# baumlin/rebvio

Hardware: AMD Instinct MI355X
Metric: frames/sec at 640x480 (~15k keylines); 1-GPU and 8-stream/8-GPU batch (higher is better)
Workload: dtype f32; 1 GPU; 640x480 synthetic stream, ~15k keylines, detect+track+IRLS pose, fp32; streams=1, keylines=14942, frames_in_hbm=24, settle_frames=995, pairs_tracked_in_window=1144, parallelism=1 independent streams, 1 per GPU, rank0_numa_node=0

## Files before the change

rebvio_amd/csrc/api.hip:

```cpp
#include <chrono>
#include <cmath>
#include <cstdio>
#include <cstdlib>
#include <cstring>
#include <limits>
#include <atomic>
#include <condition_variable>
#include <deque>
#include <map>
#include <memory>
#include <mutex>
#include <shared_mutex>
#include <thread>
#include <string>
#include <vector>

#include "common.hpp"
#include "glue.hpp"
#include "hostmath.hpp"
#include "pixel_format.hpp"

using namespace rh;

namespace {
// ... 196 lines not shown
  rebvio_hip_pair_out out;
  int keylines;
};

struct PairQueue {
  struct Step {
    rebvio_hip_map* nm[kMaxLanes];
    uint32_t seq = 0;
    int slot = -1;
    int ev_slot = -1;
  };
  Step ring[kPairSlots];
  int head = 0, count = 0;
  Step& operator[](int i) { return ring[(head + i) % kPairSlots]; }
  void push_back(const Step& st) { ring[(head + count++) % kPairSlots] = st; }
  void pop_front() {
    head = (head + 1) % kPairSlots;
    --count;
  }
  std::deque<PairRec> done;
  hipEvent_t slot_ev[kPairSlots]{};
  double t_wait = 0;
};

struct rebvio_hip_ctx {
  std::shared_ptr<LifeBlock> life = std::make_shared<LifeBlock>();
  rebvio_hip_params P{};
  KParams K{};
  int device = 0;
  hipStream_t s_det{}, s_key{}, s_trk{};
  double t_begin_enq = 0, t_begin_wait = 0;
  uint64_t t_begin_n = 0;
  std::mutex dl_mu;
  float* sa2[2][2] = {{nullptr, nullptr}, {nullptr, nullptr}};
  float* dog2[kDetPar]{};
  float* mag2[kDetPar]{};
  int* rowcount2[kDetPar]{};
  hipEvent_t ev_scan[2]{};
  hipEvent_t prev_ready[2]{};
  uint64_t launch_index = 0;
  uint64_t release_counter = 0;
  ScaleBufs sb{};
  DetectBufs db{};
  DetState* det = nullptr;
  uint64_t frame_index = 0;
  rebvio_hip_map* last_detected = nullptr;
  int widths[2][3]{};
  std::vector<rebvio_hip_map*> pool;
  float* img_dev = nullptr;
  uint8_t* img8_dev = nullptr;
  static constexpr int kPin = 16;
  void* pin[kPin]{};
  hipEvent_t pin_ev[kPin]{};
  bool pin_used[kPin]{};
  uint64_t pin_next = 0;
  int2* undist_map = nullptr;
  float* undist_img[kDetPar]{};
  uint8_t* dmask_buf = nullptr;
  const uint8_t* dmask = nullptr;
  rebvio_hip_batch* batch = nullptr;
  rebvio_hip_keyline* aos_dev = nullptr;
  int* scratch_i = nullptr;
  float* diag0 = nullptr;
  float* diag1 = nullptr;
  LmState* lm = nullptr;
  float* part = nullptr;
  float* xrv_part = nullptr;
  int* hist = nullptr;
  float* fscratch = nullptr;
  int maxblocks = 0;
  unsigned long long* lm_xch = nullptr;
  unsigned lm_tag_base = 0;
// ... 24 lines not shown
  int lm_threads = 512;
  int dm_head_form = 0;
  static constexpr int kSlots = kPairSlots;
  PairSlot* slot[kSlots]{};
  GlueRec* rec[kSlots]{};
  GlueDev* glue_dev = nullptr;
  GlueStage* glue_stage = nullptr;
  GlueState* gstate = nullptr;
  GlueState* h_gstate = nullptr;
  hm::M3 gs_R{};
  int min_pool = 0;
  int lead = 5;
  int group = 4;
  uint32_t stamp_seq = 0;
  uint32_t last_stamp = 0;
  bool forge_stamp = false;
  std::mutex pool_mu;
  std::vector<rebvio_hip_map*> frames;
  PairQueue q;
  uint64_t pair_seq = 0;
  struct DetJob {
    rebvio_hip_map* m;
    const void* img;
    int is_u8;
    const DetState* det_in;
    DetState* det_out;
    const MapState* prev_st;
    int pin_slot = -1;
    size_t pin_bytes = 0;
    int fmt = 0;
    const uint8_t* mask_static = nullptr;
    const uint8_t* mask_frame = nullptr;
  };
  std::mutex det_mu;
  std::string det_error;
  double t_detect_enq = 0, t_enq = 0, t_queued = 0;
  double t_det_launch = 0;
  uint64_t t_det_n = 0;
  bool dbg = false;
  hm::M3 wbg_shadow{};
  bool wbg_shadow_valid = false;
  bool gyro_pre_on = true;
  uint64_t t_frames = 0;
  bool owns_streams = true;
  rebvio_hip_map* bf_map[2] = {nullptr, nullptr};
  bool bf_have[2] = {false, false};
  bool bf_copy_queued[2] = {false, false};
  hipEvent_t bf_done[2]{};
  MapState* h_bf = nullptr;
  int bf_cur = 0;
  int bf_res = -1;
  bool bf_nan[2] = {false, false};
};

namespace {
void release_map(rebvio_hip_map* m, hipEvent_t done_ref = nullptr, bool record_done = true);

inline bool map_dead(const rebvio_hip_map* m) { return !m || !m->life || m->life->dead.load(std::memory_order_acquire); }
class MapAlive {
 public:
  explicit MapAlive(const rebvio_hip_map* m) : hold_(m ? m->life : nullptr) {
    if (hold_) lock_ = std::shared_lock<std::shared_mutex>(hold_->mu);
    dead_ = map_dead(m);
    if (dead_) g_err = "the map's context has been destroyed (rebvio_hip_destroy)";
  }
  bool dead() const { return dead_; }
// ... 162 lines not shown
  DetectBufs db = c->db;
  db.rowcount = c->rowcount2[b];
  if (j.pin_slot >= 0) {
    launch_copy_from_pinned(c->s_det, c->pin[j.pin_slot], const_cast<void*>(j.img), j.pin_bytes);
    HIPCHK(hipEventRecord(c->pin_ev[j.pin_slot], c->s_det));
  }
  if (c->prev_ready[b]) HIPCHK(hipStreamWaitEvent(c->s_det, c->prev_ready[b], 0));
  const void* img = j.img;
  int is_u8 = j.is_u8;
  int fmt = is_u8 ? j.fmt : 0;
  if (is_u8 && c->undist_map) {
    if (fmt == px::GRAY8)
      launch_front_end_u8(c->s_det, c->K, (const uint8_t*)img, c->undist_map, c->undist_img[b]);
    else
      launch_front_end_px(c->s_det, c->K, (const uint8_t*)img, fmt, c->undist_map, c->undist_img[b]);
    img = c->undist_img[b];
    is_u8 = 0;
    fmt = 0;
  }
  launch_scale_space(c->s_det, c->K, img, is_u8, sb, c->widths, db.rowcount, 1, fmt);
  HIPCHK(hipEventRecord(c->ev_scan[b], c->s_det));
  HIPCHK(hipStreamWaitEvent(c->s_key, c->ev_scan[b], 0));
  launch_scale_space(c->s_key, c->K, img, is_u8, sb, c->widths, db.rowcount, 2);
  if (m->has_done) HIPCHK(hipStreamWaitEvent(c->s_key, m->done_ref ? m->done_ref : m->done, 0));
  launch_keylines(c->s_key, c->K, sb, db, m->d, j.det_in, j.det_out, j.prev_st, c->widths, j.mask_static, j.mask_frame);
  HIPCHK(hipGetLastError());
  launch_df_build(c->s_key, c->K, m->d, j.det_out, true);
  HIPCHK(hipGetLastError());
  HIPCHK(hipEventRecord(m->ready, c->s_key));
  c->prev_ready[b] = m->ready;
  return 0;
}

int detect_prepare(rebvio_hip_ctx* c, const void* img_dev, int is_u8, uint64_t ts, rebvio_hip_ctx::DetJob* job, int fmt = 0,
                   const uint8_t* mask_frame = nullptr) {
  rebvio_hip_map* m = acquire_map(c);
  if (!m) return fail_msg("edge-map pool exhausted (release maps or raise map_pool)", -2);
  m->ts = ts;
  m->df_built = true;
  m->raster_order = true;
  job->m = m;
  job->img = img_dev;
  job->is_u8 = is_u8;
  job->fmt = fmt;
  job->mask_static = c->dmask;
  job->mask_frame = mask_frame;
  job->det_in = c->det + (c->frame_index % kDetRing);
  job->det_out = c->det + ((c->frame_index + 1) % kDetRing);
  job->prev_st = c->last_detected ? c->last_detected->d.st : nullptr;
  c->frame_index++;
  c->last_detected = m;
  return 0;
}

void detect_failed(rebvio_hip_ctx* c, const rebvio_hip_ctx::DetJob& job) {
  {
    std::lock_guard<std::mutex> lk(c->det_mu);
    if (c->det_error.empty()) c->det_error = g_err.empty() ? std::string("detect launch failed") : g_err;
  }
  release_map(job.m, nullptr);
}

int stage_host_frame(rebvio_hip_ctx* c, const void* img, size_t pitch_bytes, size_t row_bytes, int* slot_out, size_t* bytes_out);

int detect(rebvio_hip_ctx* c, const void* img_dev, int is_u8, int fmt, uint64_t ts, rebvio_hip_map** out, const void* host = nullptr,
           size_t pitch_bytes = 0, size_t row_bytes = 0, const uint8_t* mask_frame = nullptr) {
  {
    std::lock_guard<std::mutex> lk(c->det_mu);
    if (!c->det_error.empty()) return fail_msg(c->det_error.c_str(), -8);
  }
  rebvio_hip_ctx::DetJob job;
  int rc = host ? stage_host_frame(c, host, pitch_bytes, row_bytes, &job.pin_slot, &job.pin_bytes) : 0;
  if (rc) return rc;
  rc = detect_prepare(c, img_dev, is_u8, ts, &job, fmt, mask_frame);
  if (rc) return rc;
  const auto t0 = std::chrono::steady_clock::now();
  rc = detect_launch(c, job);
  if (c->dbg) {
    c->t_det_launch += std::chrono::duration<double, std::micro>(std::chrono::steady_clock::now() - t0).count();
    c->t_det_n++;
  }
  if (rc) {
    detect_failed(c, job);
    return rc;
  }
  *out = job.m;
  return 0;
}

void rotate_inputs(const rebvio_hip_ctx* c, const float vel[3], const float Rvel[9], const float Rback[9], float vel_r[3],
                   float Rvel_r[9]) {
  (void)c;
  const hm::M3 Rb = hm::load3(Rback);
  hm::mulv(Rb, vel, vel_r);
  hm::store3(hm::mul(hm::mul(Rb, hm::load3(Rvel)), hm::transpose(Rb)), Rvel_r);
}

void sum_xrv(const float* h_xrv, int nblocks, float Wx[36], float JtF[6], int* nm) {
  double acc[28];
  for (int k = 0; k < 28; ++k) acc[k] = 0.0;
  for (int b = 0; b < nblocks; ++b)
    for (int k = 0; k < 28; ++k) acc[k] += (double)h_xrv[(size_t)b * kXrvStride + k];
  int k = 0;
  for (int i = 0; i < 6; ++i)
    for (int j = i; j < 6; ++j) {
      Wx[i * 6 + j] = (float)acc[k];
      Wx[j * 6 + i] = (float)acc[k];
      ++k;
    }
  for (int i = 0; i < 6; ++i) JtF[i] = (float)acc[21 + i];
  if (nm) *nm = (int)std::lround(acc[27]);
}

// ... 400 lines not shown
    c->lm_persistent = std::strcmp(e, "percall") != 0;
    c->lm_spec = std::strcmp(e, "seq") != 0;
    c->lm_spec_forced = std::strcmp(e, "spec") == 0 || std::strcmp(e, "spec3") == 0;
    c->lm_spec_forced_kf = std::strcmp(e, "spec3") == 0 ? 3 : 2;
    if (std::strncmp(e, "mix", 3) == 0) c->lm_mix = std::max(1, std::atoi(e + 3));
  }
  HIPCHK(hipMalloc(&c->lm, 16 * sizeof(LmState)));
  HIPCHK(hipMemset(c->lm, 0, 16 * sizeof(LmState)));
  HIPCHK(hipMalloc(&c->part, (size_t)(kMaxLmCalls + 1) * part_call_stride(c) * sizeof(float)));
  HIPCHK(hipMemset(c->part, 0, (size_t)(kMaxLmCalls + 1) * part_call_stride(c) * sizeof(float)));
  HIPCHK(hipMalloc(&c->xrv_part, (size_t)c->maxblocks * kXrvStride * sizeof(float)));
  HIPCHK(hipMalloc(&c->hist, 128 * sizeof(int)));
  HIPCHK(hipMemset(c->hist, 0, 128 * sizeof(int)));
  HIPCHK(hipMalloc(&c->lm_zero, sizeof(LmState)));
  HIPCHK(hipMemset(c->lm_zero, 0, sizeof(LmState)));
  for (int i = 0; i < rebvio_hip_ctx::kSlots; ++i) {
    const size_t sz = sizeof(PairSlot) + (size_t)c->maxblocks * kXrvStride * sizeof(float);
    HIPCHK(hipHostMalloc(&c->slot[i], sz, hipHostMallocDefault));
    std::memset(c->slot[i], 0, sz);
    HIPCHK(hipHostMalloc(&c->rec[i], sizeof(GlueRec), hipHostMallocDefault));
    std::memset(c->rec[i], 0, sizeof(GlueRec));
    HIPCHK(hipEventCreateWithFlags(&c->q.slot_ev[i], hipEventDisableTiming));
  }
  HIPCHK(hipMalloc(&c->fscratch, 64 * sizeof(float)));
  HIPCHK(hipMalloc(&c->glue_dev, rebvio_hip_ctx::kSlots * sizeof(GlueDev)));
  HIPCHK(hipMemset(c->glue_dev, 0, rebvio_hip_ctx::kSlots * sizeof(GlueDev)));
  HIPCHK(hipMalloc(&c->glue_stage, rebvio_hip_ctx::kSlots * sizeof(GlueStage)));
  HIPCHK(hipMemset(c->glue_stage, 0, rebvio_hip_ctx::kSlots * sizeof(GlueStage)));
  HIPCHK(hipMalloc(&c->gstate, 2 * sizeof(GlueState)));
  HIPCHK(hipMemset(c->gstate, 0, 2 * sizeof(GlueState)));
  HIPCHK(hipHostMalloc(&c->h_gstate, 2 * sizeof(GlueState), hipHostMallocDefault));
  if (const char* l = std::getenv("REBVIO_HIP_LEAD")) c->lead = std::min(12, std::max(3, std::atoi(l)));
  if (const char* g = std::getenv("REBVIO_HIP_GROUP")) c->group = std::min(6, std::max(1, std::atoi(g)));
  if (const char* e = std::getenv("REBVIO_HIP_LM_THREADS")) {
    const int v = std::atoi(e);
    if (v == 256 || v == 512 || v == 1024) c->lm_threads = v;
  }
  if (const char* e = std::getenv("REBVIO_HIP_DM_HEAD"))
    c->dm_head_form = dm_form_by_name(e);
  HIPCHK(hipHostMalloc(&c->h_lm, 2 * sizeof(LmState), hipHostMallocDefault));
  HIPCHK(hipHostMalloc(&c->h_part, part_call_stride(c) * sizeof(float), hipHostMallocDefault));
  HIPCHK(hipHostMalloc(&c->h_xrv, (size_t)c->maxblocks * kXrvStride * sizeof(float), hipHostMallocDefault));
  HIPCHK(hipHostMalloc(&c->h_st, 2 * sizeof(MapState), hipHostMallocDefault));
  HIPCHK(hipHostMalloc(&c->h_f, 64 * sizeof(float), hipHostMallocDefault));

  int pool = p->map_pool > 0 ? p->map_pool : 6;
  if (pool < 4) pool = 4;
  for (int i = 0; i < pool; ++i) {
    rebvio_hip_map* m = new rebvio_hip_map;
    m->ctx = c;
    m->life = c->life;
    c->pool.push_back(m);
    int rc = alloc_map(c, m);
    if (rc) return rc;
  }
  rebvio_hip_reset_state(c);
  c->dbg = std::getenv("REBVIO_HIP_DEBUG") != nullptr;
  if (const char* e = std::getenv("REBVIO_HIP_GYRO_PRE")) c->gyro_pre_on = e[0] != '0';
  HIPCHK(hipDeviceSynchronize());
  guard.c = nullptr;
  *out = c;
  return 0;
}

void rebvio_hip_destroy(rebvio_hip_ctx* c) {
  if (!c) return;
  const std::shared_ptr<LifeBlock> life = c->life;
  std::unique_lock<std::shared_mutex> life_lk(life->mu);
  residency_remove(c->device, c);
  (void)hipSetDevice(c->device);
  if (std::getenv("REBVIO_HIP_DEBUG") && c->t_begin_n)
    std::fprintf(stderr, "[rebvio_hip] track_pair_begin over %llu pairs (us): enqueue %.1f  wait for the first half %.1f\n",
                 (unsigned long long)c->t_begin_n, c->t_begin_enq / c->t_begin_n, c->t_begin_wait / c->t_begin_n);
  (void)hipDeviceSynchronize();
  {
    std::lock_guard<std::mutex> g(g_prof.mu);
    g_prof.drain();
  }
  for (auto* m : c->frames) m->in_use = false;
  life->dead.store(true, std::memory_order_release);
  for (auto* m : c->pool) {
    free_map_device(m);
    if (!m->in_use) delete m;
  }
  c->pool.clear();
  void* dptr[] = {c->sb.a[0], c->sb.a[1], c->sb.b[0], c->sb.b[1], c->sb.dog, c->sb.mag, c->db.stash, c->db.bits,
                  c->db.rowcount, c->det, c->img_dev, c->img8_dev, c->aos_dev, c->scratch_i, c->diag0, c->diag1, c->lm,
                  c->part, c->xrv_part, c->hist, c->fscratch, c->dmask_buf};
  for (void* p : dptr)
    if (p) (void)hipFree(p);
  for (int f = 0; f < 2; ++f)
    if (c->sa2[1][f]) (void)hipFree(c->sa2[1][f]);
  void* hptr[] = {c->h_lm, c->h_part, c->h_xrv, c->h_st, c->h_f};
  for (void* p : hptr)
    if (p) (void)hipHostFree(p);
  if (c->owns_streams) {
    if (c->s_det) (void)hipStreamDestroy(c->s_det);
    if (c->s_trk) (void)hipStreamDestroy(c->s_trk);
    if (c->s_key) (void)hipStreamDestroy(c->s_key);
  }
  for (int i = 0; i < 2; ++i) {
    if (c->ev_scan[i]) (void)hipEventDestroy(c->ev_scan[i]);
  }
  for (int i = 1; i < kDetPar; ++i) {
    if (c->dog2[i]) (void)hipFree(c->dog2[i]);
    if (c->mag2[i]) (void)hipFree(c->mag2[i]);
    if (c->rowcount2[i]) (void)hipFree(c->rowcount2[i]);
  }
  for (int i = 0; i < rebvio_hip_ctx::kSlots; ++i) {
    if (c->slot[i]) (void)hipHostFree(c->slot[i]);
    if (c->rec[i]) (void)hipHostFree(c->rec[i]);
    if (c->q.slot_ev[i]) (void)hipEventDestroy(c->q.slot_ev[i]);
  }
  if (c->gstate) (void)hipFree(c->gstate);
  if (c->h_gstate) (void)hipHostFree(c->h_gstate);
  if (c->undist_map) (void)hipFree(c->undist_map);
  for (int i = 0; i < kDetPar; ++i)
    if (c->undist_img[i]) (void)hipFree(c->undist_img[i]);
  if (c->lm_xch) (void)hipFree(c->lm_xch);
  for (int i = 0; i < rebvio_hip_ctx::kPin; ++i) {
    if (c->pin[i]) (void)hipHostFree(c->pin[i]);
    if (c->pin_ev[i]) (void)hipEventDestroy(c->pin_ev[i]);
  }
  if (c->glue_dev) (void)hipFree(c->glue_dev);
  if (c->glue_stage) (void)hipFree(c->glue_stage);
// ... 93 lines not shown
}

int rebvio_hip_front_end_u8(rebvio_hip_ctx* c, const uint8_t* img, float* out) {
  HIPCHK(hipSetDevice(c->device));
  if (!c->undist_map) return fail_msg("front_end_u8: no distortion model set (rebvio_hip_set_undistort)", -3);
  const size_t Pn = (size_t)c->P.rows * c->P.cols;
  HIPCHK(hipMemcpyAsync(c->img8_dev, img, Pn, hipMemcpyHostToDevice, c->s_det));
  launch_front_end_u8(c->s_det, c->K, c->img8_dev, c->undist_map, c->undist_img[0]);
  HIPCHK(hipGetLastError());
  HIPCHK(hipMemcpyAsync(out, c->undist_img[0], Pn * sizeof(float), hipMemcpyDeviceToHost, c->s_det));
  HIPCHK(hipStreamSynchronize(c->s_det));
  return 0;
}

int rebvio_hip_front_end_px(rebvio_hip_ctx* c, const void* img, size_t pitch_bytes, int fmt, float* out) {
  int rc = check_px(c, "front_end_px", img, fmt, true, pitch_bytes);
  if (rc) return rc;
  if (!out) return fail_msg("front_end_px: null output", -3);
  HIPCHK(hipSetDevice(c->device));
  if (!c->undist_map) return fail_msg("front_end_px: no distortion model set (rebvio_hip_set_undistort)", -3);
  const size_t Pn = (size_t)c->P.rows * c->P.cols;
  const size_t rowb = (size_t)c->P.cols * px::bytes_per_pixel(fmt);
  uint8_t* stage = static_cast<uint8_t*>(u8_staging(c, fmt));
  HIPCHK(hipMemcpy2DAsync(stage, rowb, img, pitch_bytes ? pitch_bytes : rowb, rowb, (size_t)c->P.rows, hipMemcpyHostToDevice, c->s_det));
  launch_front_end_px(c->s_det, c->K, stage, fmt, c->undist_map, c->undist_img[0]);
  HIPCHK(hipGetLastError());
  HIPCHK(hipMemcpyAsync(out, c->undist_img[0], Pn * sizeof(float), hipMemcpyDeviceToHost, c->s_det));
  HIPCHK(hipStreamSynchronize(c->s_det));
  return 0;
}

int rebvio_hip_detector_state(rebvio_hip_ctx* c, float* threshold, float* auto_threshold, int* count) {
  HIPCHK(hipSetDevice(c->device));
  HIPCHK(hipStreamSynchronize(c->s_det));
  HIPCHK(hipStreamSynchronize(c->s_key));
  DetState d;
  HIPCHK(hipMemcpy(&d, c->det + (c->frame_index % kDetRing), sizeof(d), hipMemcpyDeviceToHost));
  float at = d.auto_threshold;
  if (c->last_detected) {
    MapState st;
    HIPCHK(hipMemcpy(&st, c->last_detected->d.st, sizeof(st), hipMemcpyDeviceToHost));
    if (st.n > 0) {
      float mx, mn;
      std::memcpy(&mx, &st.gmax_bits, 4);
      std::memcpy(&mn, &st.gmin_bits, 4);
      at = mx - float(kNumBins * (mx - mn)) / float(kNumBins);
    }
  }
  if (threshold) *threshold = d.threshold;
  if (auto_threshold) *auto_threshold = at;
  if (count) *count = d.count;
  return 0;
}

int rebvio_hip_map_size(rebvio_hip_map* m) {
  const MapAlive alive(m);
  if (alive.dead()) return -10;
  if (ensure_size(m)) return -1;
  return m->n_host;
}
float rebvio_hip_map_threshold(rebvio_hip_map* m) {
  const MapAlive alive(m);
  if (alive.dead()) return std::numeric_limits<float>::quiet_NaN();
  if (ensure_size(m)) return std::numeric_limits<float>::quiet_NaN();
  return m->thr_host;
}
// ... 787 lines not shown
    f.slot = slot;
    c->q.push_back(f);
    last_slot = slot;
    c->pair_seq++;
  }
  HIPCHK(hipEventRecord(c->q.slot_ev[last_slot], s));
  for (int g = 0; g < npairs; ++g) {
    c->q[c->q.count - 1 - g].ev_slot = last_slot;
    release_map(c->frames[(size_t)g], c->q.slot_ev[last_slot]);
  }
  c->frames.erase(c->frames.begin(), c->frames.begin() + npairs);
  return 0;
}

}

namespace {
int push_frame(rebvio_hip_ctx* c, const uint8_t* frame_dev, const uint8_t* frame_host, size_t host_pitch, uint64_t ts_us, rebvio_hip_pair_out* out,
               int* keylines, int fmt = 0, const uint8_t* mask_frame = nullptr) {
  rebvio_hip_map* m = nullptr;
  const auto td0 = std::chrono::steady_clock::now();
  HIPCHK(hipSetDevice(c->device));
  if (out) {
    std::memset(out, 0, sizeof(*out));
    out->status = -1;
  }
  if (keylines) *keylines = -1;
  c->min_pool = c->lead + 3 * c->group + 3;
  int rc;
  if (frame_host) {
    const size_t rowb = (size_t)c->P.cols * px::bytes_per_pixel(fmt);
    rc = detect(c, u8_staging(c, fmt), 1, fmt, ts_us, &m, frame_host, host_pitch ? host_pitch : rowb, rowb);
  } else {
    rc = detect(c, frame_dev, 1, fmt, ts_us, &m, nullptr, 0, 0, mask_frame);
  }
  if (rc) return rc;
  const auto td1 = std::chrono::steady_clock::now();
  c->t_detect_enq += std::chrono::duration<double, std::micro>(td1 - td0).count();
  c->t_frames++;
  c->frames.push_back(m);
  const int npairs = group_size((int)c->frames.size(), c->q.count, c->lead, c->group);
  if (npairs >= 1) {
    rc = stream_enqueue_group(c, npairs);
    if (rc) return rc;
  }
  c->t_enq += std::chrono::duration<double, std::micro>(std::chrono::steady_clock::now() - td1).count();
  rc = harvest(c->q, stream_lanes(c), 0);
  if (rc) return rc;
  (void)pop_records(c->q, 1, out, keylines);
  return 0;
}

}

int rebvio_hip_push_frame_u8_device(rebvio_hip_ctx* c, const uint8_t* frame_dev, uint64_t ts_us, rebvio_hip_pair_out* out,
                                    int* keylines) {
  return push_frame(c, frame_dev, nullptr, 0, ts_us, out, keylines);
}

int rebvio_hip_push_frame_u8(rebvio_hip_ctx* c, const uint8_t* frame_host, size_t pitch_bytes, uint64_t ts_us, rebvio_hip_pair_out* out,
                             int* keylines) {
  if (!frame_host) return fail_msg("push_frame_u8: null frame", -3);
  return push_frame(c, nullptr, frame_host, pitch_bytes, ts_us, out, keylines);
}

int rebvio_hip_push_frame_px_device(rebvio_hip_ctx* c, const void* frame_dev, int fmt, uint64_t ts_us, rebvio_hip_pair_out* out,
                                    int* keylines) {
// ... 80 lines not shown
                     nw, sum[8], sum[9], sum[10], sum[11], mx[11], with_open, sum[12], mx[12], sum[13], mx[13]);
        std::fprintf(stderr, "[rebvio_hip]   per wave, us mean / max:");
        for (int i = 0; i < 7; ++i) std::fprintf(stderr, "  %s %.2f / %.2f", seg[i], sum[i] * 0.01 / (double)nw, mx[i] * 0.01);
        std::fprintf(stderr, "  | slowest wave %.2f\n", slow * 0.01);
      }
    }
  } else if (c->lm_stamps && c->lm_stamp_n) {
    const int calls = (int)c->P.iterations + 1;
    std::fprintf(stderr, "[rebvio_hip] k_lm_chain workgroup 0, mean us per segment over %llu launches\n", (unsigned long long)c->lm_stamp_n);
    std::fprintf(stderr, "  prologue %.2f\n", c->lm_stamp_acc[1] / c->lm_stamp_n);
    for (int k = 0; k < calls; ++k) {
      const double* a = c->lm_stamp_acc + 1 + k * 6;
      const double n = (double)c->lm_stamp_n;
      std::fprintf(stderr, "  eval %d: collect %.2f  lm_step %.2f  evaluate %.2f  wave-reduce %.2f  carry+publish %.2f  (loop edge %.2f)\n", k,
                   a[1] / n, a[2] / n, a[3] / n, a[4] / n, a[5] / n, k + 1 < calls ? a[6] / n : 0.0);
    }
    std::fprintf(stderr, "  final collect+lm_step %.2f  forwardMatch+extRotVel %.2f\n", c->lm_stamp_acc[1 + calls * 6] / c->lm_stamp_n,
                 c->lm_stamp_acc[2 + calls * 6] / c->lm_stamp_n);
  }
  if (std::getenv("REBVIO_HIP_DEBUG") && c->t_frames) {
    const double n = (double)c->t_frames;
    std::fprintf(stderr,
                 "[rebvio_hip] host time per frame (us): detect hand-over %.1f  pair enqueue %.1f  waiting for result slots %.1f | long "
                 "directedMatch searches per pair %.0f\n",
                 c->t_detect_enq / n, c->t_enq / n, c->q.t_wait / n, c->t_queued / n);
    if (c->t_det_n)
      std::fprintf(stderr, "[rebvio_hip] detect: %.1f us of launches per frame over %llu frames\n", c->t_det_launch / (double)c->t_det_n,
                   (unsigned long long)c->t_det_n);
    c->t_detect_enq = c->t_enq = c->q.t_wait = c->t_queued = 0;
    c->t_frames = 0;
    c->t_det_launch = 0;
    c->t_det_n = 0;
  }
  int rc = 0;
  while (rc == 0 && c->frames.size() >= 2)
    rc = stream_enqueue_group(c, std::min(c->group, (int)c->frames.size() - 1));
  if (rc == 0) rc = drain(c->q, stream_lanes(c));
  for (auto* m : c->frames)
    if (m->in_use) release_map(m, nullptr);
  c->frames.clear();
  HIPCHK(hipMemsetAsync(c->hist, 0, 128 * sizeof(int), c->s_trk));
  HIPCHK(hipStreamSynchronize(c->s_det));
  HIPCHK(hipStreamSynchronize(c->s_key));
  { const int rc_ts = trk_sync(c); if (rc_ts) return rc_ts; }
  return rc;
}

int rebvio_hip_test_glue(rebvio_hip_ctx* c, const float vel[3], const float JtJ6[6], float F, float sigma_rho_min, int accept_mask,
                         const float* xrv, int n_new, float frame_dt, const float Bg[3], const float W_Bg[9], const float R_prior[9],
                         rebvio_hip_pair_out* out_dev, float* state_dev, float* second_dev, rebvio_hip_pair_out* out_host, float* state_host,
                         float* second_host) {
  HIPCHK(hipSetDevice(c->device));
  if (n_new < 0 || n_new > c->P.keylines_max) return fail_msg("test_glue: n_new out of range", -3);
  static_assert(sizeof(GlueState) == 22 * sizeof(float) && sizeof(GlueDev) == 44 * sizeof(float), "record layouts of the test hook");
  LmState lm;
  std::memset(&lm, 0, sizeof(lm));
  for (int i = 0; i < 3; ++i) lm.vel[i] = vel[i];
  for (int i = 0; i < 6; ++i) lm.JtJ[i] = JtJ6[i];
  lm.F = F;
  lm.sigma_rho_min = sigma_rho_min;
  lm.accept_mask = accept_mask;
  GlueState st;
  for (int i = 0; i < 3; ++i) st.Bg[i] = Bg[i];
  std::memcpy(st.W_Bg, W_Bg, sizeof(st.W_Bg));
  std::memcpy(st.R, R_prior, sizeof(st.R));
  st.pad = 0.f;
  const int nb = div_up(n_new, 256);
// ... 594 lines not shown
int rebvio_hip_batch_push_px_device(rebvio_hip_batch* b, const void* const* frames_dev, int fmt, uint64_t ts_us, rebvio_hip_pair_out* out,
                                    int* keylines) {
  if (!frames_dev) return fail_msg("batch_push_px_device: null frame array", -3);
  for (int l = 0; l < b->B; ++l) {
    const int rc = check_px(b->lane[l], "batch_push_px_device", frames_dev[l], fmt, false, 0);
    if (rc) return rc;
  }
  return batch_push(b, frames_dev, fmt, ts_us, out, keylines);
}

int rebvio_hip_batch_push_px_masked_device(rebvio_hip_batch* b, const void* const* frames_dev, int fmt, const uint8_t* const* masks_dev,
                                           uint64_t ts_us, rebvio_hip_pair_out* out, int* keylines) {
  if (!frames_dev) return fail_msg("batch_push_px_masked_device: null frame array", -3);
  if (!masks_dev) return fail_msg("batch_push_px_masked_device: null mask array", -3);
  for (int l = 0; l < b->B; ++l) {
    const int rc = check_px(b->lane[l], "batch_push_px_masked_device", frames_dev[l], fmt, false, 0);
    if (rc) return rc;
  }
  return batch_push(b, frames_dev, fmt, ts_us, out, keylines, masks_dev);
}

int rebvio_hip_set_detection_mask(rebvio_hip_ctx* c, const uint8_t* mask, size_t pitch_bytes) {
  const size_t rows = (size_t)c->P.rows, cols = (size_t)c->P.cols;
  if (!mask) {
    c->dmask = nullptr;
    return 0;
  }
  if (pitch_bytes != 0 && pitch_bytes < cols) {
    char buf[128];
    std::snprintf(buf, sizeof(buf), "set_detection_mask: pitch_bytes %zu below cols %zu", pitch_bytes, cols);
    return fail_msg(buf, -3);
  }
  HIPCHK(hipSetDevice(c->device));
  if (rebvio_hip_batch* b = c->batch)
    while (b->det_done_steps.load(std::memory_order_acquire) < b->step) std::this_thread::yield();
  HIPCHK(hipStreamSynchronize(c->s_key));
  if (!c->dmask_buf) HIPCHK(hipMalloc(&c->dmask_buf, rows * cols));
  HIPCHK(hipMemcpy2D(c->dmask_buf, cols, mask, pitch_bytes ? pitch_bytes : cols, cols, rows, hipMemcpyHostToDevice));
  c->dmask = c->dmask_buf;
  return 0;
}

int rebvio_hip_batch_next_records(rebvio_hip_batch* b, rebvio_hip_pair_out* out, int* keylines) { return pop_records(b->q, b->B, out, keylines); }

int rebvio_hip_batch_flush(rebvio_hip_batch* b) {
  HIPCHK(hipSetDevice(b->device));
  while (b->det_done_steps.load(std::memory_order_acquire) < b->step) std::this_thread::yield();
  if (b->dbg && b->step)
    std::fprintf(stderr, "[rebvio_hip] batch of %d lanes, host time per step (us): detect worker's launches %.1f  track enqueue %.1f  waiting "
                 "for result slots %.1f\n", b->B, (double)b->t_det_ns.load() / 1e3 / (double)b->step, b->t_trk_enq / (double)b->step,
                 b->q.t_wait / (double)b->step);
  if (b->dbg)
    std::fprintf(stderr, "[rebvio_hip] batch: pool of lane 0 holds %d maps (min_pool %d), %d steps in flight, %d detected steps queued\n",
                 (int)b->lane[0]->pool.size(), b->lane[0]->min_pool, b->q.count, (int)b->frames.size());
  int rc = 0;
  while (rc == 0 && b->frames.size() >= 2)
    rc = batch_enqueue_group(b, std::min(b->group, (int)b->frames.size() - 1));
  if (rc == 0) rc = drain(b->q, batch_lanes(b));
  for (auto& f : b->frames)
    for (size_t l = 0; l < f.m.size(); ++l) release_map(f.m[l], nullptr, l + 1 == f.m.size());
  b->frames.clear();
  for (auto* c : b->lane)
    HIPCHK(hipMemsetAsync(c->hist, 0, 128 * sizeof(int), b->st.s_trk));
  HIPCHK(hipStreamSynchronize(b->st.s_det));
  HIPCHK(hipStreamSynchronize(b->st.s_key));
  HIPCHK(hipStreamSynchronize(b->st.s_trk));
// ... 5 lines not shown
```

rebvio_amd/csrc/common.hpp:

```cpp
#pragma once

#include <hip/hip_runtime.h>
#include <cstdlib>
#include <string>
#include <stdint.h>

#include "rebvio_hip.h"

namespace rh {

constexpr int kWave = 64;
constexpr int kBlock = 256;
constexpr int kNumBins = 100;
constexpr int kMaxImageValue = 765;
constexpr unsigned kDfEmpty = 0xFFFFFFFFu;
constexpr int kDfSeqBits = 23;
constexpr unsigned kDfSeqMask = (1u << kDfSeqBits) - 1u;
constexpr int kPartStride = 16;
constexpr int kXrvStride = 32;
constexpr int kMaxLmCalls = 8;
__host__ __device__ constexpr size_t lm_xch_xrv_offset(size_t groups, size_t workgroups) {
  return ((size_t)kMaxLmCalls * groups + 1) * 16 + (2 * (size_t)kMaxLmCalls + 1) * workgroups;
}
constexpr size_t lm_xch_words(size_t groups) { return lm_xch_xrv_offset(groups, groups) + groups * (size_t)kXrvStride; }
// ... 84 lines not shown

__host__ __device__ inline int cvtt_f32(float v) {
  if (!(v >= -2147483648.0f && v < 2147483648.0f)) return (int)0x80000000;
  return (int)v;
}
__host__ __device__ inline int cvtt_f64(double v) {
  if (!(v > -2147483649.0 && v < 2147483648.0)) return (int)0x80000000;
  return (int)v;
}

struct ScaleBufs {
  float* a[2];
  float* b[2];
  float* dog;
  float* mag;
  float* scale0;
  float* scale1;
};

struct DetectBufs {
  float4* stash;
  unsigned long long* bits;
  int* rowcount;
};

void upload_tables(const float* recip128, const float* pinv75);

void launch_front_end_u8(hipStream_t s, const KParams& p, const uint8_t* src, const int2* map, float* dst);
void launch_front_end_px(hipStream_t s, const KParams& p, const uint8_t* src, int fmt, const int2* map, float* dst);
void launch_copy_from_pinned(hipStream_t s, const void* src_pinned, void* dst_dev, size_t bytes);
void launch_scale_space(hipStream_t s, const KParams& p, const void* img, int img_is_u8, const ScaleBufs& sb,
                        const int widths[2][3], int* rowcount_to_zero, int part = 3,
                        int fmt = 0 );
void launch_smooth_n(hipStream_t s, const KParams& p, const float* img, const ScaleBufs& sb, const int* widths, int n, int* rowcount_to_zero);
void launch_keylines(hipStream_t s, const KParams& p, const ScaleBufs& sb, const DetectBufs& db, const MapDev& m,
                     const DetState* det_in, DetState* det_out, const MapState* prev_st, const int widths[2][3],
                     const uint8_t* mask_static = nullptr, const uint8_t* mask_frame = nullptr );
struct DfGrid {
  int T, ntx, nty;
};
inline DfGrid df_grid(int rows, int cols) {
  DfGrid g;
  g.T = kDfTile;
  while (((cols + g.T - 1) / g.T) * ((rows + g.T - 1) / g.T) > kDfMaxTiles) g.T *= 2;
  g.ntx = (cols + g.T - 1) / g.T;
  g.nty = (rows + g.T - 1) / g.T;
  return g;
}
void launch_df_build(hipStream_t s, const KParams& p, const MapDev& m, const DetState* det_prev, bool mask_is_current);
void launch_df_decode(hipStream_t s, const KParams& p, const MapDev& m, int* id_out, int* dist_out);

void launch_rotate(hipStream_t s, const KParams& p, const MapDev& m, const float R[9], int* hist_or_null,
                   int zero_dm_counters);
void launch_quantile(hipStream_t s, const KParams& p, const MapDev& m, int* hist, float pct, int bins, float* out_dev);
void launch_try_vel(hipStream_t s, const KParams& p, const MapDev& oldm, const MapDev& newm, int mode_lm, int call,
                    int last, LmState* st_in, LmState* st_out, const float* part_prev, float* part_out, const int* hist,
                    int frame_count);
struct PairSlot {
  LmState lm;
  MapState new_st;
  MapState old_st;
  unsigned seq;
  unsigned sum;
  unsigned pad_[2];
  float xrv[1];
};
// ... 223 lines not shown
```

rebvio_amd/csrc/detect.hip:

```cpp
#include <algorithm>
#include <cstdio>
#include <cstdlib>

#include <cstring>

#include "common.hpp"
#include "pixel_format.hpp"

namespace rh {

__constant__ float c_recip[128];
__constant__ float c_pinv[75];

void upload_tables(const float* recip128, const float* pinv75) {
  (void)hipMemcpyToSymbol(HIP_SYMBOL(c_recip), recip128, sizeof(float) * 128);
  (void)hipMemcpyToSymbol(HIP_SYMBOL(c_pinv), pinv75, sizeof(float) * 75);
}

__device__ __forceinline__ float box_avg(const float* __restrict__ II, int r, int c, int d, int R, int C, int ld) {
  const int d2 = d >> 1;
  const bool top = r < d2 + 1, bot = r >= R - d2;
  const bool left = c < d2 + 1, right = c >= C - d2;
  const int r1 = (bot && !top) ? R - 1 : r + d2;
  const int c1 = (right && !left) ? C - 1 : c + d2;
// ... 322 lines not shown
#pragma unroll
    for (int k = 0; k < kBatch; ++k) {
      const int c4 = base + k * kCPP + cb;
      if (c4 < C4 && rvalid)
        reinterpret_cast<float4*>(dst)[(size_t)(r0 + lr) * C4 + c4] = *reinterpret_cast<float4*>(&tile[lr * ldw + c4 * 4]);
    }
  }
}

template <int MODE>
__global__ __launch_bounds__(256) void k_rowscan(const void* __restrict__ src0, const void* __restrict__ src1, float* __restrict__ dst0,
                                                 float* __restrict__ dst1, int R, int Cimg, int d0, int d1, int ldw) {
  rowscan_body<MODE>(src0, src1, dst0, dst1, R, Cimg, d0, d1, ldw);
}
template <int MODE>
__global__ __launch_bounds__(256) void k_rowscan_b(const LaneStatic* __restrict__ ls, LaneDynB dyn, int lane0, int stage, int R, int Cimg,
                                                   int d0, int d1, int ldw) {
  const int lane = lane0 + blockIdx.z;
  const LaneStatic& L = ls[lane];
  const bool first = stage == 0 || stage == 3;
  const void* s0 = stage == 0 ? dyn.v[lane].img
                              : (stage == 3 ? (const void*)gptr(L.undist_img[dyn.v[lane].parity]) : (stage == 1 ? (const void*)gptr(L.sa[0]) : (const void*)gptr(L.sb[0])));
  const void* s1 = first ? s0 : (stage == 1 ? (const void*)gptr(L.sa[0]) : (const void*)gptr(L.sb[1]));
  float* o0 = stage == 1 ? gptr(L.sb[0]) : gptr(L.sa[0]);
  float* o1 = first ? gptr(L.sa[0]) : (stage == 1 ? gptr(L.sb[1]) : gptr(L.sa[1]));
  if (stage == 4) {
    const int par = dyn.v[lane].parity;
    s0 = gptr(L.sb[0]);
    s1 = gptr(L.sb[1]);
    o0 = gptr(L.dog2[par]);
    o1 = gptr(L.mag2[par]);
  }
  rowscan_body<MODE>(s0, s1, o0, o1, R, Cimg, d0, d1, ldw);
}
template <int FMT>
__global__ __launch_bounds__(256) void k_rowscan_px(const void* __restrict__ src, float* __restrict__ dst, int R, int Cimg, int ldw) {
  rowscan_body<0, FMT>(src, src, dst, dst, R, Cimg, 0, 0, ldw);
}
template <int FMT>
__global__ __launch_bounds__(256) void k_rowscan_px_b(const LaneStatic* __restrict__ ls, LaneDynB dyn, int lane0, int R, int Cimg, int ldw) {
  const int lane = lane0 + blockIdx.z;
  float* o = gptr(ls[lane].sa[0]);
  rowscan_body<0, FMT>(dyn.v[lane].img, dyn.v[lane].img, o, o, R, Cimg, 0, 0, ldw);
}

constexpr int kColStrip = 16;

__device__ __forceinline__ void colscan_body(float* __restrict__ buf0, float* __restrict__ buf1, int R, int C , int ldh,
                                             int* __restrict__ zero = nullptr, int nzero = 0) {
  const uint2 vb = xcd_band_block();
  if (zero && vb.x == 0 && vb.y == 0)
    for (int i = threadIdx.x; i < nzero; i += 256) zero[i] = 0;
  extern __shared__ float4 smem4[];
  float* tile = reinterpret_cast<float*>(smem4);
  float* __restrict__ buf = vb.y ? buf1 : buf0;
  const int c0 = vb.x * kColStrip;
  const int ncols = min(kColStrip, C - c0);
  const int q = ncols >> 2;
  const int c4 = min((int)threadIdx.x & 3, q - 1);
  const bool cvalid = ((int)threadIdx.x & 3) < q;
  const int rb = (int)threadIdx.x >> 2;
  const float* gsrc = buf + c0 + c4 * 4;
  constexpr int kBatch = 4;
  constexpr int kRowsPerPass = 64;
  for (int base = 0; base < R; base += kRowsPerPass * kBatch) {
#define RH_CS_LD(k) *reinterpret_cast<const float4*>(gsrc + (size_t)min(base + (k) * kRowsPerPass + rb, R - 1) * C)
// ... 57 lines not shown
      }
    }
    for (; r < R4; r += 4) {
      float4 w = *reinterpret_cast<float4*>(colp + r);
      w.x = s + w.x;
      w.y = w.x + w.y;
      w.z = w.y + w.z;
      w.w = w.z + w.w;
      s = w.w;
      *reinterpret_cast<float4*>(colp + r) = w;
    }
    for (; r < R; ++r) {
      s = s + colp[r];
      colp[r] = s;
    }
  }
  __syncthreads();
  float* gdst = buf + c0 + c4 * 4;
  for (int base = 0; base < R; base += kRowsPerPass * kBatch) {
#pragma unroll
    for (int k = 0; k < kBatch; ++k) {
      const int r = base + k * kRowsPerPass + rb;
      if (r < R && cvalid) {
        const float* t = tile + (c4 * 4) * ldh + r;
        *reinterpret_cast<float4*>(gdst + (size_t)r * C) = make_float4(t[0], t[ldh], t[2 * ldh], t[3 * ldh]);
      }
    }
  }
}

__global__ __launch_bounds__(256) void k_colscan(float* __restrict__ buf0, float* __restrict__ buf1, int R, int C, int ldh, int* __restrict__ zero,
                                                 int nzero) {
  colscan_body(buf0, buf1, R, C, ldh, zero, nzero);
}
__global__ __launch_bounds__(256) void k_colscan_b(const LaneStatic* __restrict__ ls, int lane0, int which, int R, int C, int ldh, int zero_parity) {
  const LaneStatic& L = ls[lane0 + blockIdx.z];
  if (which == 3) {
    colscan_body(gptr(L.dog2[zero_parity]), gptr(L.mag2[zero_parity]), R, C, ldh, gptr(L.rowcount2[zero_parity]), R);
    return;
  }
  colscan_body(which == 1 ? gptr(L.sb[0]) : gptr(L.sa[0]), which == 0 ? gptr(L.sa[0]) : (which == 1 ? gptr(L.sb[1]) : gptr(L.sa[1])), R, C, ldh,
               zero_parity >= 0 ? gptr(L.rowcount2[zero_parity]) : nullptr, R);
}

constexpr int kDogMaxD = 11;
constexpr int kDogPitch = 64 + 2 + kDogMaxD + 1;
template <int kDogRows>
__device__ __forceinline__ void dog_mag_body(const float* __restrict__ II0, const float* __restrict__ II1, int d0,
                                                 int d1, float* __restrict__ dog, float* __restrict__ mag,
                                                 float* __restrict__ scale0, float* __restrict__ scale1, int R, int C,
                                                 int* __restrict__ rowcount) {
  const uint2 vb = xcd_band_block();
  constexpr int kDogTileRows = kDogRows + 2 + kDogMaxD;
  const int ld = (C + 3) & ~3;
  __shared__ float t0[kDogTileRows * kDogPitch];
  __shared__ float t1[kDogTileRows * kDogPitch];
  __shared__ float s0[kDogRows + 2][66];
  const int c0 = vb.x * 64, r0 = vb.y * kDogRows;
  const int h0 = d0 >> 1, h1 = d1 >> 1;
  const int ro0 = r0 - 2 - h0, co0 = c0 - 2 - h0, nr0 = kDogRows + 3 + 2 * h0, nc0 = 64 + 3 + 2 * h0;
  const int tx = threadIdx.x, ty = threadIdx.y;
  const int ro1 = r0 - 1 - h1, co1 = c0 - 1 - h1, nr1 = kDogRows + 1 + 2 * h1, nc1 = 64 + 1 + 2 * h1;
  constexpr int kIt = (kDogRows + 3 + kDogMaxD - 1 + 3) / 4;
  float va[kIt], vb2[kIt], wa[kIt], wb[kIt];
  const int ca0 = min(max(co0 + tx, 0), C - 1), cb0 = min(max(co0 + tx + 64, 0), C - 1);
  const int ca1 = min(max(co1 + tx, 0), C - 1), cb1 = min(max(co1 + tx + 64, 0), C - 1);
// ... 998 lines not shown
  if (part & 1) {
    if (img_is_u8 && fmt != px::GRAY8) {
      rowscan_px_attrs();
      switch (fmt) {
#define RH_RS_PX(F)                                                                                         \
  case F:                                                                                                   \
    RH_LAUNCH(k_rowscan_px<F>, g1, dim3(256), shm, s, img, sb.a[0], R, C, ldw);                               \
    break;
        RH_RS_PX(px::RGB8) RH_RS_PX(px::BGR8) RH_RS_PX(px::RGBA8) RH_RS_PX(px::BGRA8) RH_RS_PX(px::YUYV) RH_RS_PX(px::UYVY)
#undef RH_RS_PX
      }
    } else if (img_is_u8)
      RH_LAUNCH(k_rowscan<0>, g1, dim3(256), shm, s, img, img, sb.a[0], sb.a[0], R, C, 0, 0, ldw);
    else
      RH_LAUNCH(k_rowscan<1>, g1, dim3(256), shm, s, img, img, sb.a[0], sb.a[0], R, C, 0, 0, ldw);
    RH_COLSCAN(true, sb.a[0], sb.a[0]);
    RH_LAUNCH(k_rowscan<2>, g2, dim3(256), shm, s, (const void*)sb.a[0], (const void*)sb.a[0], sb.b[0], sb.b[1], R,
                       C, widths[0][0], widths[1][0], ldw);
    RH_COLSCAN(false, sb.b[0], sb.b[1]);
    RH_LAUNCH(k_rowscan<2>, g2, dim3(256), shm, s, (const void*)sb.b[0], (const void*)sb.b[1], sb.a[0], sb.a[1], R, C, widths[0][1],
              widths[1][1], ldw);
  }
  if (part == 2) {
    RH_LAUNCH(k_colscan, c2, dim3(256), cshm, s, sb.a[0], sb.a[1], R, Cp, ldh, rowcount_to_zero, R);
  } else if (part & 2) {
    RH_COLSCAN(false, sb.a[0], sb.a[1]);
    const dim3 gt(div_up(C, 64), div_up(R, kTileRowsSingle));
    RH_LAUNCH(k_dog_mag<kTileRowsSingle>, gt, dim3(64, 4), 0, s, (const float*)sb.a[0], (const float*)sb.a[1], widths[0][2], widths[1][2], sb.dog,
              sb.mag, sb.scale0, sb.scale1, R, C, rowcount_to_zero);
  }
#undef RH_COLSCAN
}

void launch_smooth_n(hipStream_t s, const KParams& p, const float* img, const ScaleBufs& sb, const int* widths, int n, int* rowcount_to_zero) {
  const int R = p.rows, C = p.cols;
  const int Cp = (C + 3) & ~3;
  const int ldw = lds_pitch(Cp);
  const size_t shm = (size_t)kStrip * ldw * sizeof(float);
  (void)hipFuncSetAttribute(reinterpret_cast<const void*>(&k_rowscan<1>), hipFuncAttributeMaxDynamicSharedMemorySize, 160 * 1024);
  (void)hipFuncSetAttribute(reinterpret_cast<const void*>(&k_rowscan<2>), hipFuncAttributeMaxDynamicSharedMemorySize, 160 * 1024);
  (void)hipFuncSetAttribute(reinterpret_cast<const void*>(&k_colscan), hipFuncAttributeMaxDynamicSharedMemorySize, 160 * 1024);
  const dim3 g1(div_up(R, kStrip), 1), c1(div_up(Cp, kColStrip), 1);
  const int ldh = lds_pitch(R + (4 - R % 4) % 4);
  const size_t cshm = (size_t)ldh * kColStrip * sizeof(float);
  float* cur = sb.a[0];
  float* other = sb.b[0];
  RH_LAUNCH(k_rowscan<1>, g1, dim3(256), shm, s, (const void*)img, (const void*)img, cur, cur, R, C, 0, 0, ldw);
  RH_LAUNCH(k_colscan, c1, dim3(256), cshm, s, cur, cur, R, Cp, ldh, (int*)nullptr, 0);
  for (int i = 0; i + 1 < n; ++i) {
    RH_LAUNCH(k_rowscan<2>, g1, dim3(256), shm, s, (const void*)cur, (const void*)cur, other, other, R, C, widths[i], widths[i], ldw);
    RH_LAUNCH(k_colscan, c1, dim3(256), cshm, s, other, other, R, Cp, ldh, (int*)nullptr, 0);
    std::swap(cur, other);
  }
  const dim3 gt(div_up(C, 64), div_up(R, kTileRowsSingle));
  RH_LAUNCH(k_dog_mag<kTileRowsSingle>, gt, dim3(64, 4), 0, s, (const float*)cur, (const float*)cur, widths[n - 1], widths[n - 1], sb.dog, sb.mag,
            sb.scale0, sb.scale1, R, C, rowcount_to_zero);
}

void launch_scale_space_b(hipStream_t s, const KParams& p, int lane0, int lanes, const LaneStatic* ls, const LaneDynB& dyn,
                          const int widths[2][3], bool lens, int fmt) {
  const int R = p.rows, C = p.cols;
  const int Cp = (C + 3) & ~3;
  const int ldw_abs = lds_pitch(Cp);
  const size_t shm = (size_t)kStrip * ldw_abs * sizeof(float);
  const int ldw = ldw_abs;
  const int ldh = lds_pitch(R + (4 - R % 4) % 4);
// ... 142 lines not shown
```

Measured before the change: 16280 frames/s.

## Batch scale-space scans for two consecutive frames into paired kernel launches

Defers a streamed frame's detection when the queue is deep enough. When the next frame arrives, the box-filter row/column scans for both frames run as single launches with a z-dimension of 2, using extra per-slot scratch buffers and rowcounts. This halves the scan launch count and doubles the grid size to fill the GPU better at 640x480. The cost is one frame of added detection latency, plus flush points in the state, finish and sync paths to launch any pending job.

```diff
diff --git a/rebvio_amd/csrc/api.hip b/rebvio_amd/csrc/api.hip
--- a/rebvio_amd/csrc/api.hip
+++ b/rebvio_amd/csrc/api.hip
@@ -252,12 +252,16 @@
   double t_begin_enq = 0, t_begin_wait = 0;
   uint64_t t_begin_n = 0;
   std::mutex dl_mu;
-  float* sa2[2][2] = {{nullptr, nullptr}, {nullptr, nullptr}};
+  float* sa2[4][2] = {{nullptr, nullptr}, {nullptr, nullptr}, {nullptr, nullptr}, {nullptr, nullptr}};
+  float* sb_b1[2] = {nullptr, nullptr};
+  int* rowcount4[4]{};
   float* dog2[kDetPar]{};
   float* mag2[kDetPar]{};
   int* rowcount2[kDetPar]{};
   hipEvent_t ev_scan[2]{};
-  hipEvent_t prev_ready[2]{};
+  hipEvent_t prev_ready[4]{};
+  uint64_t pair_launches = 0;
+  bool scan_pairs = true;
   uint64_t launch_index = 0;
   uint64_t release_counter = 0;
   ScaleBufs sb{};
@@ -348,6 +352,8 @@
     const uint8_t* mask_static = nullptr;
     const uint8_t* mask_frame = nullptr;
   };
+  DetJob pend{};
+  bool have_pend = false;
   std::mutex det_mu;
   std::string det_error;
   double t_detect_enq = 0, t_enq = 0, t_queued = 0;
@@ -576,6 +582,54 @@
   return 0;
 }
 
+int detect_launch_pair(rebvio_hip_ctx* c, const rebvio_hip_ctx::DetJob& j0, const rebvio_hip_ctx::DetJob& j1) {
+  const size_t Pp = (size_t)c->P.rows * (size_t)((c->P.cols + 3) & ~3);
+  if (!c->sa2[2][0]) {
+    for (int f = 0; f < 2; ++f) {
+      HIPCHK(hipMalloc(&c->sa2[2][f], Pp * sizeof(float)));
+      HIPCHK(hipMalloc(&c->sa2[3][f], Pp * sizeof(float)));
+      HIPCHK(hipMalloc(&c->sb_b1[f], Pp * sizeof(float)));
+    }
+    c->rowcount4[0] = c->rowcount2[0];
+    c->rowcount4[1] = c->rowcount2[1];
+    for (int i = 2; i < 4; ++i) {
+      HIPCHK(hipMalloc(&c->rowcount4[i], (size_t)c->P.rows * sizeof(int)));
+      HIPCHK(hipMemset(c->rowcount4[i], 0, (size_t)c->P.rows * sizeof(int)));
+    }
+  }
+  const int s0 = (c->pair_launches & 1) ? 2 : 0;
+  c->pair_launches++;
+  c->launch_index += 2;
+  const rebvio_hip_ctx::DetJob* const job[2] = {&j0, &j1};
+  for (int k = 0; k < 2; ++k)
+    if (c->prev_ready[s0 + k]) HIPCHK(hipStreamWaitEvent(c->s_det, c->prev_ready[s0 + k], 0));
+  const uint8_t* const img[2] = {static_cast<const uint8_t*>(j0.img), static_cast<const uint8_t*>(j1.img)};
+  float* const a[2][2] = {{c->sa2[s0][0], c->sa2[s0][1]}, {c->sa2[s0 + 1][0], c->sa2[s0 + 1][1]}};
+  float* const bb[2][2] = {{c->sb.b[0], c->sb.b[1]}, {c->sb_b1[0], c->sb_b1[1]}};
+  int* const rowcount[2] = {c->rowcount4[s0], c->rowcount4[s0 + 1]};
+  launch_scale_space_pair(c->s_det, c->K, img, a, bb, c->widths, rowcount);
+  HIPCHK(hipEventRecord(c->ev_scan[0], c->s_det));
+  HIPCHK(hipStreamWaitEvent(c->s_key, c->ev_scan[0], 0));
+  for (int k = 0; k < 2; ++k) {
+    const rebvio_hip_ctx::DetJob& j = *job[k];
+    rebvio_hip_map* m = j.m;
+    ScaleBufs sb = c->sb;
+    sb.scale0 = sb.scale1 = nullptr;
+    sb.a[0] = a[k][0];
+    sb.a[1] = a[k][1];
+    DetectBufs db = c->db;
+    db.rowcount = rowcount[k];
+    if (m->has_done) HIPCHK(hipStreamWaitEvent(c->s_key, m->done_ref ? m->done_ref : m->done, 0));
+    launch_keylines(c->s_key, c->K, sb, db, m->d, j.det_in, j.det_out, j.prev_st, c->widths, j.mask_static, j.mask_frame);
+    HIPCHK(hipGetLastError());
+    launch_df_build(c->s_key, c->K, m->d, j.det_out, true);
+    HIPCHK(hipGetLastError());
+    HIPCHK(hipEventRecord(m->ready, c->s_key));
+    c->prev_ready[s0 + k] = m->ready;
+  }
+  return 0;
+}
+
 int detect_prepare(rebvio_hip_ctx* c, const void* img_dev, int is_u8, uint64_t ts, rebvio_hip_ctx::DetJob* job, int fmt = 0,
                    const uint8_t* mask_frame = nullptr) {
   rebvio_hip_map* m = acquire_map(c);
@@ -607,22 +661,54 @@
 
 int stage_host_frame(rebvio_hip_ctx* c, const void* img, size_t pitch_bytes, size_t row_bytes, int* slot_out, size_t* bytes_out);
 
+int launch_pending(rebvio_hip_ctx* c) {
+  if (!c->have_pend) return 0;
+  c->have_pend = false;
+  const auto t0 = std::chrono::steady_clock::now();
+  const int rc = detect_launch(c, c->pend);
+  if (c->dbg) {
+    c->t_det_launch += std::chrono::duration<double, std::micro>(std::chrono::steady_clock::now() - t0).count();
+    c->t_det_n++;
+  }
+  if (rc) detect_failed(c, c->pend);
+  return rc;
+}
+
 int detect(rebvio_hip_ctx* c, const void* img_dev, int is_u8, int fmt, uint64_t ts, rebvio_hip_map** out, const void* host = nullptr,
-           size_t pitch_bytes = 0, size_t row_bytes = 0, const uint8_t* mask_frame = nullptr) {
+           size_t pitch_bytes = 0, size_t row_bytes = 0, const uint8_t* mask_frame = nullptr, bool streaming = false) {
   {
     std::lock_guard<std::mutex> lk(c->det_mu);
     if (!c->det_error.empty()) return fail_msg(c->det_error.c_str(), -8);
   }
+  const bool pairable = streaming && c->scan_pairs && !host && is_u8 && fmt == px::GRAY8 && !c->undist_map && !c->batch;
+  const bool partner = c->have_pend && pairable && (c->pend.mask_frame != nullptr) == (mask_frame != nullptr);
+  int rc = partner ? 0 : launch_pending(c);
+  if (rc) return rc;
   rebvio_hip_ctx::DetJob job;
-  int rc = host ? stage_host_frame(c, host, pitch_bytes, row_bytes, &job.pin_slot, &job.pin_bytes) : 0;
+  rc = host ? stage_host_frame(c, host, pitch_bytes, row_bytes, &job.pin_slot, &job.pin_bytes) : 0;
   if (rc) return rc;
   rc = detect_prepare(c, img_dev, is_u8, ts, &job, fmt, mask_frame);
-  if (rc) return rc;
+  if (rc) {
+    if (partner) (void)launch_pending(c);
+    return rc;
+  }
+  if (!partner && pairable && c->q.count >= c->group) {
+    c->pend = job;
+    c->have_pend = true;
+    *out = job.m;
+    return 0;
+  }
   const auto t0 = std::chrono::steady_clock::now();
-  rc = detect_launch(c, job);
+  if (partner) {
+    c->have_pend = false;
+    rc = detect_launch_pair(c, c->pend, job);
+    if (rc) detect_failed(c, c->pend);
+  } else {
+    rc = detect_launch(c, job);
+  }
   if (c->dbg) {
     c->t_det_launch += std::chrono::duration<double, std::micro>(std::chrono::steady_clock::now() - t0).count();
-    c->t_det_n++;
+    c->t_det_n += partner ? 2 : 1;
   }
   if (rc) {
     detect_failed(c, job);
@@ -1089,6 +1175,7 @@
   HIPCHK(hipHostMalloc(&c->h_gstate, 2 * sizeof(GlueState), hipHostMallocDefault));
   if (const char* l = std::getenv("REBVIO_HIP_LEAD")) c->lead = std::min(12, std::max(3, std::atoi(l)));
   if (const char* g = std::getenv("REBVIO_HIP_GROUP")) c->group = std::min(6, std::max(1, std::atoi(g)));
+  if (const char* e = std::getenv("REBVIO_HIP_SCAN_PAIRS")) c->scan_pairs = e[0] != '0';
   if (const char* e = std::getenv("REBVIO_HIP_LM_THREADS")) {
     const int v = std::atoi(e);
     if (v == 256 || v == 512 || v == 1024) c->lm_threads = v;
@@ -1146,8 +1233,13 @@
                   c->part, c->xrv_part, c->hist, c->fscratch, c->dmask_buf};
   for (void* p : dptr)
     if (p) (void)hipFree(p);
-  for (int f = 0; f < 2; ++f)
-    if (c->sa2[1][f]) (void)hipFree(c->sa2[1][f]);
+  for (int f = 0; f < 2; ++f) {
+    for (int i = 1; i < 4; ++i)
+      if (c->sa2[i][f]) (void)hipFree(c->sa2[i][f]);
+    if (c->sb_b1[f]) (void)hipFree(c->sb_b1[f]);
+  }
+  for (int i = 2; i < 4; ++i)
+    if (c->rowcount4[i]) (void)hipFree(c->rowcount4[i]);
   void* hptr[] = {c->h_lm, c->h_part, c->h_xrv, c->h_st, c->h_f};
   for (void* p : hptr)
     if (p) (void)hipHostFree(p);
@@ -1307,6 +1399,7 @@
 
 int rebvio_hip_detector_state(rebvio_hip_ctx* c, float* threshold, float* auto_threshold, int* count) {
   HIPCHK(hipSetDevice(c->device));
+  { const int rc_p = launch_pending(c); if (rc_p) return rc_p; }
   HIPCHK(hipStreamSynchronize(c->s_det));
   HIPCHK(hipStreamSynchronize(c->s_key));
   DetState d;
@@ -2160,7 +2253,7 @@
     const size_t rowb = (size_t)c->P.cols * px::bytes_per_pixel(fmt);
     rc = detect(c, u8_staging(c, fmt), 1, fmt, ts_us, &m, frame_host, host_pitch ? host_pitch : rowb, rowb);
   } else {
-    rc = detect(c, frame_dev, 1, fmt, ts_us, &m, nullptr, 0, 0, mask_frame);
+    rc = detect(c, frame_dev, 1, fmt, ts_us, &m, nullptr, 0, 0, mask_frame, true);
   }
   if (rc) return rc;
   const auto td1 = std::chrono::steady_clock::now();
@@ -2307,7 +2400,7 @@
     c->t_det_launch = 0;
     c->t_det_n = 0;
   }
-  int rc = 0;
+  int rc = launch_pending(c);
   while (rc == 0 && c->frames.size() >= 2)
     rc = stream_enqueue_group(c, std::min(c->group, (int)c->frames.size() - 1));
   if (rc == 0) rc = drain(c->q, stream_lanes(c));
@@ -2968,6 +3061,7 @@
     return fail_msg(buf, -3);
   }
   HIPCHK(hipSetDevice(c->device));
+  { const int rc_p = launch_pending(c); if (rc_p) return rc_p; }
   if (rebvio_hip_batch* b = c->batch)
     while (b->det_done_steps.load(std::memory_order_acquire) < b->step) std::this_thread::yield();
   HIPCHK(hipStreamSynchronize(c->s_key));
diff --git a/rebvio_amd/csrc/common.hpp b/rebvio_amd/csrc/common.hpp
--- a/rebvio_amd/csrc/common.hpp
+++ b/rebvio_amd/csrc/common.hpp
@@ -140,6 +140,19 @@
 void launch_scale_space(hipStream_t s, const KParams& p, const void* img, int img_is_u8, const ScaleBufs& sb,
                         const int widths[2][3], int* rowcount_to_zero, int part = 3,
                         int fmt = 0 );
+struct ScanPair {
+  const void* src0[2];
+  const void* src1[2];
+  float* dst0[2];
+  float* dst1[2];
+};
+struct ColPair {
+  float* buf0[2];
+  float* buf1[2];
+  int* zero[2];
+};
+void launch_scale_space_pair(hipStream_t s, const KParams& p, const uint8_t* const img[2], float* const a[2][2], float* const b[2][2],
+                             const int widths[2][3], int* const rowcount[2]);
 void launch_smooth_n(hipStream_t s, const KParams& p, const float* img, const ScaleBufs& sb, const int* widths, int n, int* rowcount_to_zero);
 void launch_keylines(hipStream_t s, const KParams& p, const ScaleBufs& sb, const DetectBufs& db, const MapDev& m,
                      const DetState* det_in, DetState* det_out, const MapState* prev_st, const int widths[2][3],
diff --git a/rebvio_amd/csrc/detect.hip b/rebvio_amd/csrc/detect.hip
--- a/rebvio_amd/csrc/detect.hip
+++ b/rebvio_amd/csrc/detect.hip
@@ -378,6 +378,11 @@
     o1 = gptr(L.mag2[par]);
   }
   rowscan_body<MODE>(s0, s1, o0, o1, R, Cimg, d0, d1, ldw);
+}
+template <int MODE>
+__global__ __launch_bounds__(256) void k_rowscan_p(ScanPair a, int R, int Cimg, int d0, int d1, int ldw) {
+  const int z = blockIdx.z;
+  rowscan_body<MODE>(gptr(a.src0[z]), gptr(a.src1[z]), gptr(a.dst0[z]), gptr(a.dst1[z]), R, Cimg, d0, d1, ldw);
 }
 template <int FMT>
 __global__ __launch_bounds__(256) void k_rowscan_px(const void* __restrict__ src, float* __restrict__ dst, int R, int Cimg, int ldw) {
@@ -501,6 +506,10 @@
 __global__ __launch_bounds__(256) void k_colscan(float* __restrict__ buf0, float* __restrict__ buf1, int R, int C, int ldh, int* __restrict__ zero,
                                                  int nzero) {
   colscan_body(buf0, buf1, R, C, ldh, zero, nzero);
+}
+__global__ __launch_bounds__(256) void k_colscan_p(ColPair a, int R, int C, int ldh, int nzero) {
+  const int z = blockIdx.z;
+  colscan_body(gptr(a.buf0[z]), gptr(a.buf1[z]), R, C, ldh, gptr(a.zero[z]), nzero);
 }
 __global__ __launch_bounds__(256) void k_colscan_b(const LaneStatic* __restrict__ ls, int lane0, int which, int R, int C, int ldh, int zero_parity) {
   const LaneStatic& L = ls[lane0 + blockIdx.z];
@@ -1565,6 +1574,37 @@
 #undef RH_COLSCAN
 }
 
+void launch_scale_space_pair(hipStream_t s, const KParams& p, const uint8_t* const img[2], float* const a[2][2], float* const b[2][2],
+                             const int widths[2][3], int* const rowcount[2]) {
+  const int R = p.rows, C = p.cols;
+  const int Cp = (C + 3) & ~3;
+  const int ldw = lds_pitch(Cp);
+  const size_t shm = (size_t)kStrip * ldw * sizeof(float);
+  const int ldh = lds_pitch(R + (4 - R % 4) % 4);
+  const size_t cshm = (size_t)ldh * kColStrip * sizeof(float);
+  static bool attr_done = false;
+  if (!attr_done) {
+    (void)hipFuncSetAttribute(reinterpret_cast<const void*>(&k_rowscan_p<0>), hipFuncAttributeMaxDynamicSharedMemorySize, 160 * 1024);
+    (void)hipFuncSetAttribute(reinterpret_cast<const void*>(&k_rowscan_p<2>), hipFuncAttributeMaxDynamicSharedMemorySize, 160 * 1024);
+    (void)hipFuncSetAttribute(reinterpret_cast<const void*>(&k_colscan_p), hipFuncAttributeMaxDynamicSharedMemorySize, 160 * 1024);
+    attr_done = true;
+  }
+  const dim3 g1(div_up(R, kStrip), 1, 2), g2(div_up(R, kStrip), 2, 2);
+  const dim3 c1(div_up(Cp, kColStrip), 1, 2), c2(div_up(Cp, kColStrip), 2, 2);
+  const ScanPair r1{{img[0], img[1]}, {img[0], img[1]}, {a[0][0], a[1][0]}, {a[0][0], a[1][0]}};
+  RH_LAUNCH(k_rowscan_p<0>, g1, dim3(256), shm, s, r1, R, C, 0, 0, ldw);
+  const ColPair q1{{a[0][0], a[1][0]}, {a[0][0], a[1][0]}, {nullptr, nullptr}};
+  RH_LAUNCH(k_colscan_p, c1, dim3(256), cshm, s, q1, R, Cp, ldh, 0);
+  const ScanPair r2{{a[0][0], a[1][0]}, {a[0][0], a[1][0]}, {b[0][0], b[1][0]}, {b[0][1], b[1][1]}};
+  RH_LAUNCH(k_rowscan_p<2>, g2, dim3(256), shm, s, r2, R, C, widths[0][0], widths[1][0], ldw);
+  const ColPair q2{{b[0][0], b[1][0]}, {b[0][1], b[1][1]}, {nullptr, nullptr}};
+  RH_LAUNCH(k_colscan_p, c2, dim3(256), cshm, s, q2, R, Cp, ldh, 0);
+  const ScanPair r3{{b[0][0], b[1][0]}, {b[0][1], b[1][1]}, {a[0][0], a[1][0]}, {a[0][1], a[1][1]}};
+  RH_LAUNCH(k_rowscan_p<2>, g2, dim3(256), shm, s, r3, R, C, widths[0][1], widths[1][1], ldw);
+  const ColPair q3{{a[0][0], a[1][0]}, {a[0][1], a[1][1]}, {rowcount[0], rowcount[1]}};
+  RH_LAUNCH(k_colscan_p, c2, dim3(256), cshm, s, q3, R, Cp, ldh, R);
+}
+
 void launch_smooth_n(hipStream_t s, const KParams& p, const float* img, const ScaleBufs& sb, const int* widths, int n, int* rowcount_to_zero) {
   const int R = p.rows, C = p.cols;
   const int Cp = (C + 3) & ~3;
```

Measured after the change: 16260 frames/s (median of 2 runs). No clear change (-0.1%).
